# k2-fsa/Flow2GAN

Hardware: AMD Instinct MI355X
Metric: audio-seconds/sec (train step, G+D fwd/bwd) mel_24k_base (higher is better)
Workload: dtype f32 (fp32-class products on the bf16 matrix pipe for the long reductions and the direct MRD convs: every fp32 operand as three bf16 pieces = 24 significand bits, the six v_mfma_f32_32x32x16_bf16 products with i + j <= 2 per fp32 product, fp32 accumulate, error <= 2^-23 per product; short reductions ; 1 GPU; mel_24k_base GAN stage-2 train step: D-step + G-step, each on its own batch (MPD+MRD+FM+multi-scale mel), fwd+bwd+grad all-reduce, no optimizer (metric is fwd/bwd); per_gpu_batch=64, gan=gan_multi_scale_mel_recon, parallelism=dp1, optimizer=none

## Files before the change

### flow2gan_amd/_lib.py

```python
from __future__ import annotations

import ctypes as C
import os

import torch

_HERE = os.path.dirname(os.path.abspath(__file__))
LIB_PATH = os.environ.get("F2G_LIB_PATH") or os.path.join(_HERE, "libflow2gan_hip.so")

c_float_p = C.c_void_p


class Operand(C.Structure):
    _fields_ = [
        ("base", C.c_void_p), ("rows", C.c_int32), ("cols", C.c_int32),
        ("P1", C.c_int32), ("P0", C.c_int32), ("seglen", C.c_int32),
        ("step1", C.c_int32), ("pad1", C.c_int32), ("L1", C.c_int32),
        ("step0", C.c_int32), ("pad0", C.c_int32), ("unit", C.c_int32), ("L0u", C.c_int32),
        ("seq_stride", C.c_int64), ("line_stride", C.c_int64),
        ("reflect", C.c_int32), ("split", C.c_int32),
        ("alpha", C.c_void_p), ("lrelu_src", C.c_void_p),
        ("lrelu_slope", C.c_float), ("unbounded", C.c_int32),
    ]


class Epilogue(C.Structure):
    _fields_ = [
        ("C", C.c_void_p), ("ldc", C.c_int64), ("P0o", C.c_int32), ("c_bf16", C.c_int32),
        ("seq_stride_o", C.c_int64), ("row_stride_o", C.c_int64), ("off_o", C.c_int64),
        ("bias", C.c_void_p), ("res", C.c_void_p), ("ldres", C.c_int64), ("gamma", C.c_void_p),
        ("aux", C.c_void_p), ("ldaux", C.c_int64), ("alpha_n", C.c_void_p),
        ("colsum_alpha", C.c_void_p), ("colsum", C.c_void_p),
        ("lrelu_slope", C.c_float), ("scale", C.c_float),
        ("accumulate", C.c_int32), ("atomic", C.c_int32),
        ("prelu_slope", C.c_void_p), ("prelu_out", C.c_void_p), ("ld_prelu_out", C.c_int64),
        ("mask_src", C.c_void_p), ("fm_ref", C.c_void_p), ("fm_wdev", C.c_void_p),
        ("mask_slope", C.c_float), ("fm_w", C.c_float),
        ("x3_out", C.c_void_p), ("colsum_part_ld", C.c_int64),
    ]


class MultiEntry(C.Structure):
    _fields_ = [("out", C.c_void_p), ("inp", C.c_void_p), ("kind", C.c_int32), ("blocks", C.c_int32),
                ("n", C.c_int32 * 4), ("s", C.c_int64 * 4)]


MULTI_MAX = 48


class MultiDesc(C.Structure):
    _fields_ = [("n", C.c_int32), ("_pad", C.c_int32), ("e", MultiEntry * MULTI_MAX)]


class GemmDesc(C.Structure):
    _fields_ = [("A", Operand), ("B", Operand), ("E", Epilogue), ("form", C.c_int32),
                ("split_k", C.c_int32), ("precision", C.c_int32), ("_pad3", C.c_int32)]


class DwnormFwd(C.Structure):
    _fields_ = [
        ("x", C.c_void_p), ("ldx", C.c_int64), ("z", C.c_void_p), ("ldz", C.c_int64),
        ("B", C.c_int32), ("F", C.c_int32), ("C", C.c_int32), ("K", C.c_int32),
        ("lens", C.c_void_p), ("w_dw", C.c_void_p), ("b_dw", C.c_void_p), ("beta", C.c_void_p),
        ("log_scale", C.c_void_p), ("cproj", C.c_void_p), ("ldcp", C.c_int64),
        ("Fc", C.c_int32), ("up", C.c_int32), ("te", C.c_void_p), ("ldte", C.c_int64),
        ("rstd", C.c_void_p), ("z_format", C.c_int32), ("_pad", C.c_int32),
    ]


class DwnormBwd(C.Structure):
    _fields_ = [
# ... 128 lines not shown
    "f2g_period_fold_bwd": [_P, _P, _I, _I, _I, _I, _I],
    "f2g_fill": [_P, _F, _L],
    "f2g_bucket_arm": [_P, _L, C.c_int32],
    "f2g_scale": [_P, _F, _L],
    "f2g_log_clip": [_P, _L, _F],
    "f2g_conv32_s2_fwd": [C.POINTER(Conv32Desc)],
    "f2g_conv32_s2_dgrad": [C.POINTER(Conv32Desc)],
    "f2g_conv33_fwd": [C.POINTER(Conv32Desc)],
    "f2g_conv33_wgrad": [C.POINTER(Conv32Desc), _P],
    "f2g_conv32_s2_wgrad": [C.POINTER(Conv32Desc), _P],
    "f2g_conv2ch_fwd": [C.POINTER(Conv2chDesc)],
    "f2g_conv2ch_wgrad": [C.POINTER(Conv2chDesc)],
    "f2g_conv2ch_dgrad": [C.POINTER(Conv2chDesc)],
    "f2g_convpost_fwd": [C.POINTER(Conv2chDesc)],
    "f2g_convpost_wgrad": [C.POINTER(Conv2chDesc)],
    "f2g_convpost_dgrad": [C.POINTER(Conv2chDesc)],
    "f2g_wave_stats": [_P, _L, _L, _I, _I, _P, _P],
    "f2g_wave_gain": [_P, _L, _P, _L, _L, _I, _I, _I, _P, _P, _P],
    "f2g_sadam_stats": [_P, _P, _I, _P, _I],
    "f2g_sadam_prepare": [_P, C.POINTER(SadamGroup), _P, _P, _P, _P],
    "f2g_lrelu_bwd_colsum": [_P, _P, _P, _F, _P, _F, _I, _I, _L, _P],
    "f2g_zero_halo": [_P, _I, _I, _I, _I, _I],
    "f2g_sadam_update": [_P, _P, _I, _P],
    "f2g_mlp_pack": [_P, _P, _L, _P, _L, _I, _I],
    "f2g_fused_mlp": [C.POINTER(FusedMlpDesc)],
    "f2g_fused_block": [C.POINTER(DwnormFwd), C.POINTER(FusedMlpDesc)],
    "f2g_fused_block_multi": [C.POINTER(DwnormFwd), C.POINTER(FusedMlpDesc), C.c_int32],
    "f2g_istft_ola_multi": [C.POINTER(OlaMultiDesc), _P, _I, _I, _F, _I],
    "f2g_split_bf16x3": [_P, _P, _L, _I, _I],
    "f2g_multi": [C.POINTER(MultiDesc)],
}
EXPORTS = sorted(list(_SIGS) + ["f2g_version", "f2g_last_error", "f2g_gemm_last_path", "f2g_gemm_last_kernel",
                                 "f2g_fused_last_launch",
                                 "f2g_gemm_lean_ok", "f2g_gemm_wgrad_lean", "f2g_fused_mlp_ok",
                                 "f2g_dwnorm_bwd_workspace", "f2g_split_bf16x3_bytes", "f2g_gemm_x6_ok",
                                 "f2g_gemm_colsum_part_rows", "f2g_set_option", "f2g_get_option",
                                 "f2g_dwconv_bwd_workspace", "f2g_sadam_chunk_elems"])


class F2GError(RuntimeError):
    pass


def _load():
    if not os.path.exists(LIB_PATH):
        raise ImportError(
            f"{LIB_PATH} is missing: build it with `python -c 'import __graft_entry__ as g; "
            "g.build()'` (or `make -C flow2gan_amd/csrc`). There is no CPU fallback.")
    lib = C.CDLL(LIB_PATH)
    for name, args in _SIGS.items():
        fn = getattr(lib, name)
        fn.argtypes = list(args) + [C.c_void_p]
        fn.restype = C.c_int
    for name in ("f2g_dwnorm_bwd_workspace", "f2g_dwconv_bwd_workspace"):
        fn = getattr(lib, name)
        fn.argtypes = [C.c_int32] * 4
        fn.restype = C.c_int64
    lib.f2g_gemm_lean_ok.argtypes = [C.POINTER(GemmDesc)]
    lib.f2g_gemm_lean_ok.restype = C.c_int
    lib.f2g_gemm_wgrad_lean.argtypes = [C.POINTER(GemmDesc)]
    lib.f2g_gemm_wgrad_lean.restype = C.c_int
    lib.f2g_split_bf16x3_bytes.argtypes = [C.c_int32, C.c_int32]
    lib.f2g_split_bf16x3_bytes.restype = C.c_int64
    lib.f2g_gemm_x6_ok.argtypes = [C.POINTER(GemmDesc)]
    lib.f2g_gemm_x6_ok.restype = C.c_int
    lib.f2g_gemm_colsum_part_rows.argtypes = [C.POINTER(GemmDesc)]
    lib.f2g_gemm_colsum_part_rows.restype = C.c_int32
    lib.f2g_fused_mlp_ok.argtypes = [C.c_int32, C.c_int32]
    lib.f2g_fused_mlp_ok.restype = C.c_int
    lib.f2g_sadam_chunk_elems.argtypes = []
    lib.f2g_sadam_chunk_elems.restype = C.c_int32
    lib.f2g_set_option.argtypes = [C.c_char_p, C.c_int32]
    lib.f2g_set_option.restype = C.c_int
    lib.f2g_get_option.argtypes = [C.c_char_p, C.POINTER(C.c_int32)]
    lib.f2g_get_option.restype = C.c_int
    lib.f2g_version.restype = C.c_char_p
    lib.f2g_last_error.restype = C.c_char_p
    lib.f2g_gemm_last_kernel.argtypes = []
    lib.f2g_gemm_last_kernel.restype = C.c_char_p
    lib.f2g_fused_last_launch.argtypes = []
    lib.f2g_fused_last_launch.restype = C.c_char_p
    return lib


lib = _load()


def version() -> str:
    return lib.f2g_version().decode()


def set_option(name: str, value: int) -> int:
    old = C.c_int32()
    if lib.f2g_get_option(name.encode(), C.byref(old)) or lib.f2g_set_option(name.encode(), int(value)):
# ... 45 lines not shown
```

### flow2gan_amd/csrc/capi.hip

```cpp
#include <stdio.h>
#include <stdlib.h>
#include <string.h>
#include <strings.h>

#include <mutex>

#include "common.h"
#include "version_gen.h"

static char g_err[256] = "";

void f2g_set_error(const char* msg) {
  strncpy(g_err, msg ? msg : "", sizeof(g_err) - 1);
  g_err[sizeof(g_err) - 1] = 0;
}

int f2g_check_launch() {
  hipError_t e = hipGetLastError();
  if (e != hipSuccess) {
    f2g_set_error(hipGetErrorString(e));
    return F2G_ELAUNCH;
  }
  return F2G_OK;
}

extern "C" const char* f2g_version(void) { return "flow2gan_hip 0.4.0 src:" F2G_SRC_HASH " gfx950"; }
extern "C" const char* f2g_last_error(void) { return g_err; }

namespace {
struct Opt { const char* name; int value; };
Opt g_opts[F2G_OPT_COUNT] = {
    {"lean_tall", 1}, {"lean_wgrad", 1}, {"x6p", 1}, {"deterministic", 0}, {"streamk", 1}, {"mlp_rt", 0},
    {"mlp_split", 0}, {"multi_rt384", 4}, {"multi_rt512", 3}, {"streamk_min", 4}};
std::once_flag g_opts_once;

int opt_index(const char* name, size_t len) {
  for (int i = 0; i < F2G_OPT_COUNT; ++i)
    if (strlen(g_opts[i].name) == len && strncasecmp(g_opts[i].name, name, len) == 0) return i;
  return -1;
}

void opts_init() {
  const char* e = getenv("F2G_OPTS");
  while (e && *e) {
    const char* end = strchr(e, ',');
    const size_t len = end ? (size_t)(end - e) : strlen(e);
    const char* eq = (const char*)memchr(e, '=', len);
    if (eq) {
      const int i = opt_index(e, (size_t)(eq - e));
      if (i >= 0) g_opts[i].value = atoi(eq + 1);
    }
    e = end ? end + 1 : nullptr;
  }
  const char* det = getenv("F2G_DETERMINISTIC");
  if (det) g_opts[F2G_OPT_DETERMINISTIC].value = atoi(det) != 0;
}
}

int f2g_opt(int id) {
  std::call_once(g_opts_once, opts_init);
  return g_opts[id].value;
}

extern "C" int f2g_set_option(const char* name, int32_t value) {
  std::call_once(g_opts_once, opts_init);
  const int i = name ? opt_index(name, strlen(name)) : -1;
// ... 16 lines not shown
```

### flow2gan_amd/csrc/common.h

```cpp
#pragma once
#include <hip/hip_runtime.h>
#include <stdint.h>

#include <type_traits>

#include "../../include/flow2gan_hip.h"

int f2g_check_launch();
void f2g_note_kernel(const char* name, int split, int path);
enum f2g_opt_id {
  F2G_OPT_LEAN_TALL,
  F2G_OPT_LEAN_WGRAD,
  F2G_OPT_X6P,
  F2G_OPT_DETERMINISTIC,
  F2G_OPT_STREAMK,
  F2G_OPT_MLP_RT,
  F2G_OPT_MLP_SPLIT,
  F2G_OPT_MULTI_RT384,
  F2G_OPT_MULTI_RT512,
  F2G_OPT_STREAMK_MIN,
  F2G_OPT_COUNT
};
int f2g_opt(int id);
int f2g_gemm_narrow(const f2g_gemm_desc& d, hipStream_t st);
void f2g_set_error(const char* msg);
int f2g_x6p_ok(const f2g_gemm_desc& d, int taps);
int f2g_launch_x6p(const f2g_gemm_desc& d, int taps, long long a_extent, hipStream_t st);
int f2g_leanw6t_ok(const f2g_gemm_desc& d, int split);
int f2g_launch_leanw6t(const f2g_gemm_desc& d, int split, hipStream_t st);
struct f2g_colsegs {
  float* out[3];
  int begin[3];
  int count[3];
};
int f2g_colsum_segments(const float* a, long long lda, int rows, int ncols,
                        const f2g_colsegs& segs, hipStream_t st);

#define F2G_WAVE 64

__device__ __forceinline__ float wave_sum(float v) {
#pragma unroll
  for (int o = 32; o > 0; o >>= 1) v += __shfl_xor(v, o);
  return v;
}

__device__ __forceinline__ float wave_max(float v) {
#pragma unroll
  for (int o = 32; o > 0; o >>= 1) v = fmaxf(v, __shfl_xor(v, o));
  return v;
}

typedef float f2g_f32x2 __attribute__((ext_vector_type(2)));
typedef __bf16 f2g_bf16x2 __attribute__((ext_vector_type(2)));
// ... 26 lines not shown
```

### flow2gan_amd/csrc/gemm.hip

```cpp
#include <hip/hip_runtime.h>
#include <stddef.h>
#include <stdint.h>
#include <stdio.h>
#include <string.h>

#include "gemm_common.h"

namespace {

int g_last_path = 0;
const char* g_last_kernel = "";
int g_last_split = 1;

struct RowCtx {
  long long base;
  int l1b, e0;
};

__device__ __forceinline__ RowCtx decode_row(const f2g_operand& S, int r) {
  RowCtx rc;
  int s, p1, p0;
  if (S.P0 == 1 && S.P1 == 1) {
    s = r; p1 = 0; p0 = 0;
  } else {
// ... 720 lines not shown
extern "C" int f2g_to_bf16(void* dst, const float* src, int64_t n, f2g_stream_t stream) {
  if (!dst || !src || (n & 3) || (((uintptr_t)dst) & 7) || !al16(src)) return F2G_EINVAL;
  if (n == 0) return F2G_OK;
  const long long n4 = n / 4;
  long long blocks = (n4 + 255) / 256;
  if (blocks > 256 * 16) blocks = 256 * 16;
  hipLaunchKernelGGL(to_bf16_kernel, dim3((unsigned)blocks), dim3(256), 0, (hipStream_t)stream,
                     reinterpret_cast<uint2*>(dst), reinterpret_cast<const float4*>(src), n4);
  return f2g_check_launch();
}

extern "C" int f2g_split_bf16(float* dst, const float* src, int64_t n, f2g_stream_t stream) {
  if (!dst || !src || (n & 3) || !al16(dst) || !al16(src)) return F2G_EINVAL;
  if (n == 0) return F2G_OK;
  const long long n4 = n / 4;
  long long blocks = (n4 + 255) / 256;
  if (blocks > 256 * 16) blocks = 256 * 16;
  hipLaunchKernelGGL(split_bf16_kernel, dim3((unsigned)blocks), dim3(256), 0, (hipStream_t)stream,
                     reinterpret_cast<uint4*>(dst), reinterpret_cast<const float4*>(src), n4);
  return f2g_check_launch();
}

extern "C" int f2g_gemm(const f2g_gemm_desc* dp, f2g_stream_t stream) {
  if (!dp || !dp->A.base || !dp->B.base || !dp->E.C) return F2G_EINVAL;
  f2g_note_kernel("", 1, g_last_path);
  const f2g_gemm_desc& d = *dp;
  hipStream_t st = (hipStream_t)stream;
  int split = d.split_k > 0 ? d.split_k : 1;
  if (d.E.colsum_part_ld > 0 && f2g_gemm_colsum_part_rows(dp) == 0) {
    f2g_set_error("f2g_gemm: E.colsum_part_ld needs a precision-3 launch with the wide epilogue "
                  "(f2g_gemm_colsum_part_rows(d) == 0 for this descriptor)");
    return F2G_EINVAL;
  }
  if (d.precision == 3 && d.form == 2) {
    if (d.A.split || d.B.split || d.A.rows != d.B.rows || !f2g_leanw_ok(d) || d.E.x3_out ||
        (split > 1 && !d.E.atomic)) {
      f2g_set_error("f2g_gemm precision 3, form 2: fp32 operands the K-major weight-gradient kernel reads");
      return F2G_EINVAL;
    }
    return f2g_launch_leanw(d, 6, split, st);
  }
  if (d.precision == 3) return f2g_gemm_x6(d, st);
  if (d.E.x3_out) {
    f2g_set_error("f2g_gemm: E.x3_out belongs to precision 3");
    return F2G_EINVAL;
  }
  {
    const int nr = f2g_gemm_narrow(d, st);
    if (nr != 0) return nr < 0 ? nr : F2G_OK;
    f2g_note_kernel("", 1, 0);
  }
  if (d.E.prelu_slope && (d.E.atomic || d.E.accumulate || d.E.P0o > 0 || d.form == 2)) return F2G_EINVAL;
  if (d.E.mask_src && (d.E.atomic || d.E.accumulate || d.form == 2)) return F2G_EINVAL;
  if (d.form == 0 || d.form == 1) {
    const bool f1 = d.form == 1;
    if (f1 ? d.A.cols != d.B.rows : d.A.cols != d.B.cols) return F2G_EINVAL;
    if (!host_plain(d.B)) return F2G_EINVAL;
    const int M = d.A.rows, N = f1 ? d.B.cols : d.B.rows, K = d.A.cols;
    const int am = op_mode(d.A, true), bm = op_mode(d.B, !f1);
    const bool linear = d.E.lrelu_slope == 0.f && d.E.res != d.E.C && d.E.aux != d.E.C && !d.E.prelu_slope &&
                        !d.E.mask_src;
    int s = d.split_k;
    const bool no_auto = f2g_opt(F2G_OPT_DETERMINISTIC) != 0;
    const bool presplit = d.A.split != 0 && d.B.split == d.A.split;
    const bool bf16img = d.A.split == 2;
    const bool lean = !f1 && N > 64 && f2g_lean_operands_ok(d) &&
                      (d.precision == 0 || ((d.precision == 1 || d.precision == 2) && presplit)) &&
                      (!bf16img || (d.precision == 2 && f2g_lean_bf16_ok(d)));
    if ((d.A.split || d.B.split) && !(lean && d.precision != 0)) return F2G_EINVAL;
// ... 52 lines not shown
```

### flow2gan_amd/csrc/gemm_common.h

```cpp
#pragma once
#include "common.h"

bool f2g_lean_operands_ok(const f2g_gemm_desc& d);
bool f2g_lean_bf16_ok(const f2g_gemm_desc& d);
int f2g_lean_stream_k(int M, int N, int K, bool all_grids);
int f2g_launch_lean(const f2g_gemm_desc& d, int M, int N, int K, int split, int upb, hipStream_t st);
bool f2g_leanw_ok(const f2g_gemm_desc& d);
bool f2g_leanw_fp32_takes(const f2g_gemm_desc& d, int split);
int f2g_launch_leanw(const f2g_gemm_desc& d, int pieces, int split, hipStream_t st);
int f2g_gemm_x6(const f2g_gemm_desc& d, hipStream_t st);

#ifndef F2G_LABVAR
#define F2G_LABVAR 0
#endif
#ifndef F2G_X6LAB
#define F2G_X6LAB 0
#endif
#if F2G_X6LAB & 1
#define X6LAB_EPI if (acc[0][0][0] == 1.2345e30f)
#else
#define X6LAB_EPI
#endif
#if F2G_X6LAB & 2
#define X6LAB_X3 acc[0][0][1] == 1.2345e30f &&
#else
#define X6LAB_X3
#endif
#if F2G_X6LAB & 256
#define X6PROF_STAMP(t) asm volatile("s_memtime %0" : "=s"(t) : : "memory")
#define X6PROF_ACC(sum, t1, t0)                                                                              \
  {                                                                                                          \
    unsigned dt_;                                                                                            \
    asm volatile("s_sub_u32 %0, %1, %2" : "=s"(dt_) : "s"((unsigned)(t1)), "s"((unsigned)(t0)) : "memory"); \
    sum += dt_;                                                                                              \
  }
#else
#define X6PROF_STAMP(t)
#define X6PROF_ACC(sum, t1, t0)
#endif

namespace {

// ... 140 lines not shown
```

### flow2gan_amd/csrc/gemm_wgrad.hip

```cpp
#include <stddef.h>
#include <stdint.h>

#include "gemm_common.h"

namespace {


template <bool BWIN>
__global__ __launch_bounds__(256, 2)
void gemm_leanw3_kernel(const f2g_gemm_desc d, int M, int N, int K, int kchunk) {
  constexpr int PL = 32 * 256;
  constexpr int BUF = 4 * PL;
  extern __shared__ __attribute__((aligned(16))) float smem[];
  unsigned char* sm = reinterpret_cast<unsigned char*>(smem);
  const int tid = threadIdx.x, lane = tid & 63, wave = tid >> 6;
  const int wm = wave >> 1, wn = wave & 1, li = lane & 31, h = lane >> 5;
  int m0, n0;
  tile_of_block(128, 128, m0, n0);
  const int kbeg = blockIdx.z * kchunk;
  int kend = kbeg + kchunk;
  if (kend > K) kend = K;
  const int nt = (kend - kbeg + BK - 1) / BK;
  if (nt <= 0) return;

// ... 451 lines not shown
  return (long long)(B.rows / B.P0) * B.seq_stride * 4 < 0x7ff00000ll;
}

bool f2g_leanw_fp32_takes(const f2g_gemm_desc& d, int split) {
  const int leanw_mode = f2g_opt(F2G_OPT_LEAN_WGRAD);
  if (d.form != 2 || d.A.split || d.B.split || split < 1) return false;
  return leanw_mode > 0 && d.precision == 0 && d.E.atomic && f2g_leanw_ok(d) &&
         (host_plain(d.B) || d.B.P0 >= 16) && (leanw_mode > 1 || d.A.rows / split >= 4096);
}

template <auto KPLAIN, auto KWIN, int SMEM, int PATH>
static int launch_leanw(const f2g_gemm_desc& d, const char* plain_name, const char* win_name, int split,
                        hipStream_t st) {
  const int M = d.A.cols, N = d.B.cols, K = d.A.rows;
  int kchunk = ((K + split - 1) / split + BK - 1) / BK * BK;
  const int zs = (K + kchunk - 1) / kchunk;
  dim3 grid(M / 128, N / 128, zs);
  dyn_lds_once<KPLAIN, KWIN>(SMEM);
  const bool plain = host_plain(d.B);
  f2g_note_kernel(plain ? plain_name : win_name, split, PATH);
  hipLaunchKernelGGL(plain ? KPLAIN : KWIN, grid, dim3(256), SMEM, st, d, M, N, K, kchunk);
  return f2g_check_launch();
}

int f2g_launch_leanw(const f2g_gemm_desc& d, int pieces, int split, hipStream_t st) {
  if (pieces == 1)
    return launch_leanw<gemm_leanw_kernel<false>, gemm_leanw_kernel<true>, 2 * 2 * 32 * 128 * 4, 1>(
        d, "leanw<bwin=0>", "leanw<bwin=1>", split, st);
  if (pieces == 3)
    return launch_leanw<gemm_leanw3_kernel<false>, gemm_leanw3_kernel<true>, 2 * 4 * 32 * 256, 1>(
        d, "leanw3<bwin=0>", "leanw3<bwin=1>", split, st);
  if (f2g_leanw6t_ok(d, split))
    return f2g_launch_leanw6t(d, split, st);
  return launch_leanw<gemm_leanw6_kernel<false>, gemm_leanw6_kernel<true>, 6 * 32 * 256, 4>(
      d, "leanw6<bwin=0>", "leanw6<bwin=1>", split, st);
}

extern "C" int f2g_gemm_wgrad_lean(const f2g_gemm_desc* dp) {
  if (!dp || !dp->A.base || !dp->B.base) return 0;
  return f2g_leanw_fp32_takes(*dp, dp->split_k < 1 ? 1 : dp->split_k) ? 1 : 0;
}
```

### flow2gan_amd/fused.py

```python
from __future__ import annotations

import os
import random
from typing import List, Optional

import torch

from . import ops
from .models.modules import dft_matrices
from .ops import gemm, mat, win1d

LIMIT_PROB = 0.6


def _limit_draw(training: bool) -> bool:
    return bool(training and random.random() < LIMIT_PROB)


def frames_lens(audio_lens_cpu: Optional[List[int]], hop: int, device):
    if audio_lens_cpu is None:
        return None
    return torch.tensor([1 + int(l) // hop for l in audio_lens_cpu], dtype=torch.int32,
                        device=device)

# ... 93 lines not shown
    zsplit = 1 if fmt == 1 else 0
    z = ops.empty(rows, Cc, device=dev)
    ops.dwnorm_fwd(x, z, B, F, Cc, bp.K, lens, bp.w_dw, bp.b_dw, bp.beta, bp.log_scale.reshape(1),
                   cproj, ldcp, Fc, up, cp_off, te, ldte, te_off, z_format=zsplit)
    a = ops.empty(rows, Hh, device=dev)
    if keep:
        p = ops.empty(rows, Hh, device=dev)
        share = ops.split_sharing(z, p)
        with share:
            gemm(mat(z, rows, Cc, split=zsplit), mat(bp.w1.reshape(Hh, Cc)), a, bias=bp.b1,
                 prelu=bp.alpha, prelu_out=p)
            out = ops.empty(rows, Cc, device=dev)
            gemm(mat(p, rows, Hh), mat(bp.w2.reshape(Cc, Hh)), out, bias=bp.b2, res=x,
                 gamma=bp.gamma.reshape(Cc))
        return out, z, (a, p, share, zsplit)
    p = a
    gemm(mat(z, rows, Cc, split=zsplit), mat(bp.w1.reshape(Hh, Cc)), a, bias=bp.b1, prelu=bp.alpha)
    out = ops.empty(rows, Cc, device=dev)
    gemm(mat(p, rows, Hh), mat(bp.w2.reshape(Cc, Hh)), out, bias=bp.b2, res=x,
         gamma=bp.gamma.reshape(Cc))
    return out, z, (a, p, None, zsplit)


def block_bwd(bp: _Blk, x, z, a, gout, B, F, lens, limit_norm: bool, limit_scale: bool,
              cproj=None, ldcp=0, Fc=0, up=1, cp_off=0, te=None, ldte=0, te_off=0, g_cproj=None,
              g_te=None, g_cproj_store=False):
    a, p_act, share, zsplit = a
    if share is None:
        share = ops.split_sharing()
    dev = x.device
    rows, Cc, Hh = B * F, bp.C, bp.H
    (g_w2, g_b2, g_alpha, g_b1, g_w1, g_beta, g_ls, g_wdw, g_bdw, g_gamma) = ops.zeros_many(
        [(Cc, Hh), (Cc,), (Hh,), (Hh,), (Hh, Cc), (Cc,), (1,), (Cc, 1, bp.K), (Cc,), (Cc, 1)], dev)
    ops.colsum(g_b2, gout, rows, Cc)
    with share, ops.split_sharing(gout):
        ops.wgrad(gout, Cc, gout.stride(0), mat(p_act, rows, Hh), g_w2)
        gemm(mat(gout, rows, Cc), mat(bp.w2.reshape(Cc, Hh)), a, form=1, aux=a, alpha_n=bp.alpha,
             colsum_alpha=g_alpha, colsum=g_b1)
    with share, ops.split_sharing(a):
        ops.wgrad(a, Hh, a.stride(0), mat(z, rows, Cc, split=zsplit), g_w1)
        gemm(mat(a, rows, Hh), mat(bp.w1.reshape(Hh, Cc)), z, form=1)
    share.drop()
    du = ops.empty(rows, Cc, device=dev)
    ops.dwnorm_bwd(x, z, du, B, F, Cc, bp.K, lens, bp.w_dw, bp.b_dw, bp.beta,
                   bp.log_scale.reshape(1), cproj, ldcp, Fc, up, cp_off, te, ldte, te_off,
                   g_cproj=g_cproj, g_te=g_te, g_beta=g_beta, g_log_scale=g_ls,
                   g_cproj_store=g_cproj_store)
    gx = ops.empty(rows, Cc, device=dev)
    ops.dwconv_bwd(du, x, gx, B, F, Cc, bp.K, lens, bp.w_dw, gres=gout, gamma=bp.gamma.reshape(Cc),
                   g_w=g_wdw, g_b=g_bdw, g_gamma=g_gamma)
    if limit_norm:
        ops.limit_grad(g_ls, bp.log_scale.reshape(1), -1.5, 1.5)
    if limit_scale:
        ops.limit_grad(g_gamma, bp.gamma, 0.5, 1.0)
    grads = [g_wdw, g_bdw, g_ls.reshape(()), g_beta, g_w1.reshape(Hh, Cc, 1), g_b1, g_alpha,
             g_w2.reshape(Cc, Hh, 1), g_b2, g_gamma]
    return gx, grads


def cond_encoder_params(enc) -> list:
    p = [enc.in_proj.weight, enc.in_proj.bias, enc.in_norm.log_scale, enc.in_norm.bias]
    for blk in enc.blocks:
        p += block_params(blk)
    return p


class CondEncoderFn(GradAwareFunction):

    @staticmethod
# ... 758 lines not shown
```

### flow2gan_amd/ops.py

```python
from __future__ import annotations

import ctypes as C
from typing import Optional

import torch

from . import _lib as L
from ._opts import opt
from ._lib import DwconvBwd, DwnormBwd, DwnormFwd, Epilogue, GemmDesc, Operand, call, ptr


def empty(*shape, device, dtype=torch.float32):
    return torch.empty(*shape, device=device, dtype=dtype)


def zeros(*shape, device):
    t = torch.empty(*shape, device=device, dtype=torch.float32)
    fill_(t, 0.0)
    return t


def fill_(t, v: float):
    if BATCH is not None and t.numel() > 0:
        import struct
# ... 325 lines not shown
    o.lrelu_slope = slope
    o.unbounded = 1 if (unbounded and offset == 0 and t.is_contiguous()
                        and t.numel() == nseq * o.seq_stride) else 0
    o._keep = (t, lrelu_src)
    return o


def win2d(t, nseq: int, H: int, W: int, Cin: int, W_out: int, kh: int, kw: int, stride_w: int,
          pad_h: int, pad_w: int, line_stride: Optional[int] = None,
          seq_stride: Optional[int] = None, offset: int = 0, lrelu_src=None,
          slope: float = 0.0) -> Operand:
    o = Operand()
    o.base = ptr(t) + 4 * offset
    o.rows, o.cols = nseq * H * W_out, kh * kw * Cin
    o.P1, o.P0 = H, W_out
    o.seglen = kw * Cin
    o.step1, o.pad1, o.L1 = 1, pad_h, H
    o.step0, o.pad0, o.unit, o.L0u = stride_w, pad_w, Cin, W * Cin
    o.line_stride = line_stride if line_stride is not None else W * Cin
    o.seq_stride = seq_stride if seq_stride is not None else H * o.line_stride
    o.reflect = 0
    o.alpha = None
    o.lrelu_src = None if lrelu_src is None else ptr(lrelu_src) + 4 * offset
    o.lrelu_slope = slope
    o._keep = (t, lrelu_src)
    return o


def gemm(A: Operand, Bm: Operand, out, form: int = 0, ldc: Optional[int] = None, *, bias=None,
         res=None, ldres: Optional[int] = None, gamma=None, aux=None, ldaux: Optional[int] = None,
         alpha_n=None, colsum_alpha=None, colsum=None, lrelu: float = 0.0, scale: float = 0.0,
         accumulate: bool = False, atomic: bool = False, split_k: int = 0, out_offset: int = 0,
         rowmap=None, prelu=None, prelu_out=None, mask=None, fm=None, x3_out: bool = False,
         true_k: Optional[int] = None, true_n: Optional[int] = None):
    if form == 1:
        src = getattr(Bm, "_src", None)
        if src is not None and src.shape[0] % 32 == 0 and src.shape[1] > 64:
            Bm, form = mat(transposed(src)), 0
    d = GemmDesc()
    d.A, d.B = A, Bm
    e = Epilogue()
    e.C = ptr(out) + 4 * out_offset
    e.ldc = ldc if ldc is not None else out.stride(0)
    e.c_bf16 = 1 if out.dtype == torch.bfloat16 else 0
    if rowmap is not None:
        e.P0o, e.seq_stride_o, e.row_stride_o, e.off_o = rowmap
    else:
        e.P0o = 0
    e.bias = ptr(bias)
    e.res = ptr(res)
    e.ldres = ldres if ldres is not None else (res.stride(0) if res is not None else 0)
    e.gamma = ptr(gamma)
    e.aux = ptr(aux)
    e.ldaux = ldaux if ldaux is not None else (aux.stride(0) if aux is not None else 0)
    e.alpha_n = ptr(alpha_n)
    e.colsum_alpha = ptr(colsum_alpha)
    e.colsum = ptr(colsum)
    e.lrelu_slope = lrelu
    e.scale = scale
    e.accumulate = 1 if accumulate else 0
    e.atomic = 1 if atomic else 0
    e.prelu_slope = ptr(prelu)
    e.prelu_out = ptr(prelu_out)
    e.ld_prelu_out = prelu_out.stride(0) if prelu_out is not None else 0
    if mask is not None:
        e.mask_src = ptr(mask[0]) + 4 * mask[1]
        e.mask_slope = float(mask[2])
        if fm is not None:
            e.fm_ref = ptr(fm[0]) + 4 * fm[1]
            e.fm_w = float(fm[2])
            e.fm_wdev = ptr(fm[3])
    d.E = e
    d.form = form
    if split_k == -1:
        tiles = ((A.cols + 127) // 128) * ((Bm.cols + 127) // 128)
        split_k = split_for(A.rows, tiles)
        if form == 2 and GEMM_PRECISION == 0 and atomic:
            d.split_k, d.precision = split_k, 0
            if L.lib.f2g_gemm_wgrad_lean(C.byref(d)):
                split_k = split_for(A.rows, tiles, True)
    d.split_k = split_k
    d.precision = GEMM_PRECISION
    if GEMM_PRECISION == 3:
        d.precision = 0
        in_kernel = X6F == 1
        if X6F == 2 and X6F_MIN_K <= A.cols < X6_MIN_K and (
                (Bm.rows >= X6F_MIN_N and ((A.rows + 127) // 128) * ((Bm.rows + 127) // 128) >= X6F_MIN_TILES)
                or (A.rows >= X6F_TALL_ROWS and Bm.rows >= 128)):
            in_kernel = True
        if X6F == 2 and 128 <= A.cols < X6_MIN_K and A.rows >= X6F_TALL_ROWS and Bm.rows == 32:
            in_kernel = True
        if X6F == 2 and X6_MIN_K <= A.cols < X6_NOPASS_K and A.P0 == 1 and A.P1 == 1 and not _is_const(A._keep[0]):
            in_kernel = True
        if form == 0 and A.split == 0 and Bm.split == 0 and A.rows >= X6_MIN_ROWS \
                and (A.cols >= X6_MIN_K or in_kernel) and not atomic \
                and split_k <= 1 and out.dtype == torch.float32 and _x3_window_ok(A):
            buf = getattr(out, "_f2g_x3_buf", None) if x3_out else None
            if buf is not None and X6F != 1 and not getattr(out, "_f2g_x3_bad", False) \
                    and out_offset % 32 == 0 and prelu_out is None:
                d.E.x3_out = ptr(buf) + (out_offset // 32) * 192
            how = L.lib.f2g_gemm_x6_ok(C.byref(d))
            if not how and d.E.x3_out:
                d.E.x3_out = None
                how = L.lib.f2g_gemm_x6_ok(C.byref(d))
            if how:
                if in_kernel and not (how & 4):
                    in_kernel = False
                    how = how if A.cols >= X6_MIN_K else 0
                if how:
                    if not in_kernel:
                        d.A, d.B = _x3_operand(A), _x3_operand(Bm)
                    elif Bm.P0 == 1 and Bm.P1 == 1 and _is_const(Bm._keep[0]):
                        d.B = _x3_operand(Bm, frag_major=X6G and Bm.rows % 32 == 0 and Bm.rows > 32)
                    d.precision = 3
            if d.precision != 3:
                d.E.x3_out = None
        if form == 2 and atomic and A.split == 0 and Bm.split == 0 and A.lrelu_src is None \
                and A.rows >= X6_MIN_K and L.lib.f2g_gemm_lean_ok(C.byref(d)):
            d.precision = 3
        if x3_out:
            if d.E.x3_out:
                out._f2g_x3 = out._f2g_x3_buf
            else:
                out._f2g_x3_bad = True
    if (GEMM_PRECISION == 1 and form in (0, 2)) or (GEMM_PRECISION == 2 and form == 0):
        ok = L.lib.f2g_gemm_lean_ok(C.byref(d))
        if GEMM_PRECISION == 2 and (ok & 2):
            d.A, d.B = _bf16_operand(A), _bf16_operand(Bm)
        elif ok:
            d.A, d.B = _split_operand(A), _split_operand(Bm)
    parts = None
    if COLSUM_PARTS and d.precision == 3 and form == 0 and (colsum is not None or colsum_alpha is not None) \
            and A.rows >= COLSUM_PARTS_MIN_ROWS:
        nrows = L.lib.f2g_gemm_colsum_part_rows(C.byref(d))
        if nrows > 0:
            ncol = Bm.rows
            both = colsum is not None and colsum_alpha is not None
            parts = torch.empty(nrows, (2 if both else 1) * ncol, device=out.device, dtype=torch.float32)
            d.E.colsum_part_ld = parts.stride(0)
            if colsum_alpha is not None:
                d.E.colsum_alpha = ptr(parts)
            if colsum is not None:
                d.E.colsum = ptr(parts) + (4 * ncol if both else 0)
    if GEMM_TIMER is not None:
        GEMM_TIMER.launch(d, A, Bm, form, true_k, true_n)
    else:
        call("f2g_gemm", C.byref(d))
    if parts is not None:
        nrows, ncol = parts.shape[0], Bm.rows
        if colsum is not None and colsum_alpha is not None and ptr(colsum) == ptr(colsum_alpha) + 4 * ncol:
            call("f2g_colsum", ptr(colsum_alpha), ptr(parts), parts.stride(0), None, 0, nrows, 2 * ncol)
            return out
# ... 594 lines not shown
    def join(self):
        if not self.on:
            return
        for s in self.streams:
            ev = torch.cuda.Event()
            ev.record(s)
            self.main.wait_event(ev)


def split_for(reduction_rows: int, out_tiles: int, two_per_cu: bool = False) -> int:
    slabs = max(1, reduction_rows // 32)
    smax = max(1, min(512, slabs // 16))
    R = 256
    if two_per_cu:
        R = 512
        smax = max(1, min(smax, reduction_rows // 4096))
    cands = set(range(1, min(smax, 64) + 1))
    for m in range(1, 9):
        s = (R * m) // out_tiles
        if 1 <= s <= smax:
            cands.add(s)

    def fill(s):
        b = out_tiles * s
        return b / (((b + R - 1) // R) * R)

    best = max(fill(s) for s in cands)
    pair = [s for s in cands if out_tiles * s <= 512 and fill(s) >= best - 0.05]
    if pair:
        return max(pair)
    return min(s for s in cands if fill(s) >= best - 0.02)


def wgrad(dY, M: int, ldy: int, X: Operand, g_out, ldg: Optional[int] = None, out_offset: int = 0,
          dy_lrelu_src=None, slope: float = 0.0):
    rows = X.rows
    A = mat(dY, rows, M, ldy, lrelu_src=dy_lrelu_src, slope=slope)
    gemm(A, X, g_out, form=2, ldc=ldg, atomic=True, split_k=-1, out_offset=out_offset)


def fused_mlp_applies(Cc: int, Hh: int) -> bool:
    return GEMM_PRECISION == 2 and bool(L.lib.f2g_fused_mlp_ok(Cc, Hh))


def mlp_pack(w1, w2):
    def build(ts):
        a, b = ts
        Hh, Cc = a.shape[0], a.shape[1]
        out = torch.empty(2 * Cc * Hh, device=a.device, dtype=torch.bfloat16)
        call("f2g_mlp_pack", ptr(out), ptr(a), Cc, ptr(b), Hh, Cc, Hh)
        return out
    return derived_multi([w1, w2], "mlp_pack", build)


def fused_mlp(z, wp, b1, alpha, b2, res, gamma, out, rows: int, Cc: int, Hh: int, parts: int = 0):
    d = L.FusedMlpDesc()
    d.parts = parts
    d.z, d.ldz, d.wp = ptr(z), z.stride(0), ptr(wp)
    d.b1, d.alpha, d.b2 = ptr(b1), ptr(alpha), ptr(b2)
    d.res, d.ldres, d.gamma = ptr(res), (res.stride(0) if res is not None else 0), ptr(gamma)
    d.out, d.ldo = ptr(out), out.stride(0)
    d.rows, d.C, d.H = rows, Cc, Hh
    if GEMM_TIMER is not None:
        GEMM_TIMER.time(lambda: call("f2g_fused_mlp", C.byref(d)), 4.0 * rows * Cc * Hh,
                        (0, rows, Cc, 2 * Hh), path="fused-mlp")
    else:
        call("f2g_fused_mlp", C.byref(d))
    return out


def fused_block(x, B, F, Cc, K, lens, w_dw, b_dw, beta, log_scale, wp, b1, alpha, b2, gamma, out,
# ... 495 lines not shown
```

### include/flow2gan_hip.h

```cpp
#ifndef FLOW2GAN_HIP_H
#define FLOW2GAN_HIP_H

#include <stdint.h>

#ifdef __cplusplus
extern "C" {
#endif

typedef void* f2g_stream_t;

enum {
  F2G_OK = 0,
  F2G_EINVAL = -1,
  F2G_ELAUNCH = -2,
};

const char* f2g_version(void);
const char* f2g_last_error(void);

int f2g_set_option(const char* name, int32_t value);
int f2g_get_option(const char* name, int32_t* value);

typedef struct {
  const float* base;
// ... 10 lines not shown
  float lrelu_slope;
  int32_t unbounded;
} f2g_operand;

typedef struct {
  float* C;
  int64_t ldc;
  int32_t P0o;
  int32_t c_bf16;
  int64_t seq_stride_o, row_stride_o, off_o;
  const float* bias;
  const float* res;
  int64_t ldres;
  const float* gamma;
  const float* aux;
  int64_t ldaux;
  const float* alpha_n;
  float* colsum_alpha;
  float* colsum;
  float lrelu_slope;
  float scale;
  int32_t accumulate;
  int32_t atomic;
  const float* prelu_slope;
  float* prelu_out;
  int64_t ld_prelu_out;
  const float* mask_src;
  const float* fm_ref;
  const float* fm_wdev;
  float mask_slope;
  float fm_w;
  void* x3_out;
  int64_t colsum_part_ld;
} f2g_epilogue;

typedef struct {
  f2g_operand A, B;
  f2g_epilogue E;
  int32_t form;
  int32_t split_k;
  int32_t precision;
  int32_t _pad3;
} f2g_gemm_desc;

int f2g_gemm(const f2g_gemm_desc* d, f2g_stream_t stream);
int f2g_gemm_wgrad_lean(const f2g_gemm_desc* d);
int f2g_gemm_lean_ok(const f2g_gemm_desc* d);
int f2g_split_bf16(float* dst, const float* src, int64_t n, f2g_stream_t stream);
int f2g_to_bf16(void* dst, const float* src, int64_t n, f2g_stream_t stream);
int64_t f2g_split_bf16x3_bytes(int32_t rows, int32_t K);
int f2g_split_bf16x3(void* dst, const float* src, int64_t ld, int32_t rows, int32_t K, f2g_stream_t stream);
int f2g_gemm_x6_ok(const f2g_gemm_desc* d);
int32_t f2g_gemm_colsum_part_rows(const f2g_gemm_desc* d);

int f2g_gemm_last_path(void);
const char* f2g_gemm_last_kernel(void);

typedef struct {
  const float* x;
  int64_t ldx;
  float* z;
  int64_t ldz;
  int32_t B, F, C, K;
  const int32_t* lens;
  const float* w_dw;
  const float* b_dw;
  const float* beta;
  const float* log_scale;
  const float* cproj;
  int64_t ldcp;
  int32_t Fc, up;
  const float* te;
  int64_t ldte;
  float* rstd;
  int32_t z_format;
  int32_t _pad;
} f2g_dwnorm_fwd_desc;
int f2g_dwnorm_fwd(const f2g_dwnorm_fwd_desc* d, f2g_stream_t stream);

// ... 303 lines not shown
```

Measured before the change: 786.5 audio-s/s.

## Add wide-tile bf16x3 weight-gradient kernel with fused A column-sum

Adds a new weight-gradient GEMM kernel that uses larger output tiles (256x256 or 192x384 per 512-thread block) with in-kernel three-way bf16 splitting, LDS double buffering and six MFMA products per fp32 product. It also folds the bias-gradient column sum of dY into the kernel, so the MLP backward no longer runs a separate colsum pass over gout. Split-K is re-chosen from the wide tile count. The aim is more operand reuse per load and one fewer read of dY, at the cost of higher register and LDS use per block (launch bounds of one block) and atomic adds on the outputs.

Result: no change. 791.1 audio-s/s (median of 6 runs) (+0.6%).

```diff
diff --git a/flow2gan_amd/_lib.py b/flow2gan_amd/_lib.py
--- a/flow2gan_amd/_lib.py
+++ b/flow2gan_amd/_lib.py
@@ -36,7 +36,7 @@
         ("prelu_slope", C.c_void_p), ("prelu_out", C.c_void_p), ("ld_prelu_out", C.c_int64),
         ("mask_src", C.c_void_p), ("fm_ref", C.c_void_p), ("fm_wdev", C.c_void_p),
         ("mask_slope", C.c_float), ("fm_w", C.c_float),
-        ("x3_out", C.c_void_p), ("colsum_part_ld", C.c_int64),
+        ("x3_out", C.c_void_p), ("colsum_part_ld", C.c_int64), ("colsum_a", C.c_void_p),
     ]
 
 
@@ -231,7 +231,7 @@
 }
 EXPORTS = sorted(list(_SIGS) + ["f2g_version", "f2g_last_error", "f2g_gemm_last_path", "f2g_gemm_last_kernel",
                                  "f2g_fused_last_launch",
-                                 "f2g_gemm_lean_ok", "f2g_gemm_wgrad_lean", "f2g_fused_mlp_ok",
+                                 "f2g_gemm_lean_ok", "f2g_gemm_wgrad_lean", "f2g_gemm_wgrad_wide", "f2g_fused_mlp_ok",
                                  "f2g_dwnorm_bwd_workspace", "f2g_split_bf16x3_bytes", "f2g_gemm_x6_ok",
                                  "f2g_gemm_colsum_part_rows", "f2g_set_option", "f2g_get_option",
                                  "f2g_dwconv_bwd_workspace", "f2g_sadam_chunk_elems"])
@@ -259,6 +259,8 @@
     lib.f2g_gemm_lean_ok.restype = C.c_int
     lib.f2g_gemm_wgrad_lean.argtypes = [C.POINTER(GemmDesc)]
     lib.f2g_gemm_wgrad_lean.restype = C.c_int
+    lib.f2g_gemm_wgrad_wide.argtypes = [C.POINTER(GemmDesc)]
+    lib.f2g_gemm_wgrad_wide.restype = C.c_int32
     lib.f2g_split_bf16x3_bytes.argtypes = [C.c_int32, C.c_int32]
     lib.f2g_split_bf16x3_bytes.restype = C.c_int64
     lib.f2g_gemm_x6_ok.argtypes = [C.POINTER(GemmDesc)]
diff --git a/flow2gan_amd/csrc/capi.hip b/flow2gan_amd/csrc/capi.hip
--- a/flow2gan_amd/csrc/capi.hip
+++ b/flow2gan_amd/csrc/capi.hip
@@ -31,7 +31,8 @@
 struct Opt { const char* name; int value; };
 Opt g_opts[F2G_OPT_COUNT] = {
     {"lean_tall", 1}, {"lean_wgrad", 1}, {"x6p", 1}, {"deterministic", 0}, {"streamk", 1}, {"mlp_rt", 0},
-    {"mlp_split", 0}, {"multi_rt384", 4}, {"multi_rt512", 3}, {"streamk_min", 4}};
+    {"mlp_split", 0}, {"multi_rt384", 4}, {"multi_rt512", 3}, {"streamk_min", 4},
+    {"wgrad_wide", 1}};
 std::once_flag g_opts_once;
 
 int opt_index(const char* name, size_t len) {
diff --git a/flow2gan_amd/csrc/common.h b/flow2gan_amd/csrc/common.h
--- a/flow2gan_amd/csrc/common.h
+++ b/flow2gan_amd/csrc/common.h
@@ -19,6 +19,7 @@
   F2G_OPT_MULTI_RT384,
   F2G_OPT_MULTI_RT512,
   F2G_OPT_STREAMK_MIN,
+  F2G_OPT_WGRAD_WIDE,
   F2G_OPT_COUNT
 };
 int f2g_opt(int id);
diff --git a/flow2gan_amd/csrc/gemm.hip b/flow2gan_amd/csrc/gemm.hip
--- a/flow2gan_amd/csrc/gemm.hip
+++ b/flow2gan_amd/csrc/gemm.hip
@@ -776,9 +776,14 @@
                   "(f2g_gemm_colsum_part_rows(d) == 0 for this descriptor)");
     return F2G_EINVAL;
   }
+  if (d.E.colsum_a && !(d.precision == 3 && d.form == 2 && f2g_leanw6w_tiles(d, split) > 0)) {
+    f2g_set_error("f2g_gemm: E.colsum_a needs a launch the wide weight-gradient kernel takes "
+                  "(f2g_gemm_wgrad_wide(d) > 0 for this descriptor)");
+    return F2G_EINVAL;
+  }
   if (d.precision == 3 && d.form == 2) {
-    if (d.A.split || d.B.split || d.A.rows != d.B.rows || !f2g_leanw_ok(d) || d.E.x3_out ||
-        (split > 1 && !d.E.atomic)) {
+    if (d.A.split || d.B.split || d.A.rows != d.B.rows || d.E.x3_out || (split > 1 && !d.E.atomic) ||
+        (!f2g_leanw_ok(d) && f2g_leanw6w_tiles(d, split) == 0)) {
       f2g_set_error("f2g_gemm precision 3, form 2: fp32 operands the K-major weight-gradient kernel reads");
       return F2G_EINVAL;
     }
diff --git a/flow2gan_amd/csrc/gemm_common.h b/flow2gan_amd/csrc/gemm_common.h
--- a/flow2gan_amd/csrc/gemm_common.h
+++ b/flow2gan_amd/csrc/gemm_common.h
@@ -8,6 +8,8 @@
 bool f2g_leanw_ok(const f2g_gemm_desc& d);
 bool f2g_leanw_fp32_takes(const f2g_gemm_desc& d, int split);
 int f2g_launch_leanw(const f2g_gemm_desc& d, int pieces, int split, hipStream_t st);
+int f2g_leanw6w_tiles(const f2g_gemm_desc& d, int split);
+int f2g_launch_leanw6w(const f2g_gemm_desc& d, int split, hipStream_t st);
 int f2g_gemm_x6(const f2g_gemm_desc& d, hipStream_t st);
 
 #ifndef F2G_LABVAR
diff --git a/flow2gan_amd/csrc/gemm_wgrad.hip b/flow2gan_amd/csrc/gemm_wgrad.hip
--- a/flow2gan_amd/csrc/gemm_wgrad.hip
+++ b/flow2gan_amd/csrc/gemm_wgrad.hip
@@ -507,6 +507,8 @@
         d, "leanw3<bwin=0>", "leanw3<bwin=1>", split, st);
   if (f2g_leanw6t_ok(d, split))
     return f2g_launch_leanw6t(d, split, st);
+  if (f2g_leanw6w_tiles(d, split) > 0)
+    return f2g_launch_leanw6w(d, split, st);
   return launch_leanw<gemm_leanw6_kernel<false>, gemm_leanw6_kernel<true>, 6 * 32 * 256, 4>(
       d, "leanw6<bwin=0>", "leanw6<bwin=1>", split, st);
 }
diff --git a/flow2gan_amd/csrc/gemm_wgrad_wide.hip b/flow2gan_amd/csrc/gemm_wgrad_wide.hip
--- /dev/null
+++ b/flow2gan_amd/csrc/gemm_wgrad_wide.hip
@@ -0,0 +1,204 @@
+#include <stddef.h>
+#include <stdint.h>
+
+#include "gemm_common.h"
+
+namespace {
+
+template <int TM, int TN>
+__global__ __launch_bounds__(512, 1) void gemm_leanw6w_kernel(const f2g_gemm_desc d, int K, int kchunk) {
+  constexpr int BMT = 64 * TM, BNT = 128 * TN;
+  constexpr int PA = (BMT + 127) / 128, PB = BNT / 128;
+  constexpr int PLB = 16 * 256;
+  constexpr int OFFB = PA * 3 * PLB;
+  constexpr int BUFB = (PA + PB) * 3 * PLB;
+  extern __shared__ __attribute__((aligned(16))) unsigned char smw[];
+  const int tid = threadIdx.x, lane = tid & 63, wave = tid >> 6;
+  const int wm = wave >> 2, wn = wave & 3, li = lane & 31, h = lane >> 5;
+  int m0, n0;
+  tile_of_block(BMT, BNT, m0, n0);
+  const int kbeg = blockIdx.z * kchunk;
+  int kend = kbeg + kchunk;
+  if (kend > K) kend = K;
+  const int nt = (kend - kbeg + 15) / 16;
+  if (nt <= 0) return;
+  __amdgpu_buffer_rsrc_t ra = __builtin_amdgcn_make_buffer_rsrc(
+      (void*)d.A.base, 0, (unsigned)((long long)K * d.A.seq_stride * 4), 0x00020000);
+  __amdgpu_buffer_rsrc_t rb = __builtin_amdgcn_make_buffer_rsrc(
+      (void*)d.B.base, 0, (unsigned)((long long)K * d.B.seq_stride * 4), 0x00020000);
+  const int cc = tid & 31, r0 = tid >> 5;
+  const unsigned offA = (unsigned)(((long long)r0 * d.A.seq_stride + m0 + 4 * cc) * 4);
+  const unsigned offB = (unsigned)(((long long)r0 * d.B.seq_stride + n0 + 4 * cc) * 4);
+  const int rowA = (int)(d.A.seq_stride * 4), rowB = (int)(d.B.seq_stride * 4);
+  const int wof = r0 * 256 + ((((cc >> 3) ^ (r0 & 3))) << 6) + (cc & 7) * 8;
+  const int g4 = lane >> 4, i16 = lane & 15;
+  const int rrow = (g4 >> 1) * 8 + (i16 >> 2), within = (g4 & 1) * 32 + (i16 & 3) * 8;
+  int rofA[TM], rofB[TN];
+#pragma unroll
+  for (int mi = 0; mi < TM; ++mi) {
+    const int cb = wm * TM + mi;
+    rofA[mi] = (cb >> 2) * 3 * PLB + rrow * 256 + ((((cb & 3) ^ (rrow & 3))) << 6) + within;
+  }
+#pragma unroll
+  for (int ni = 0; ni < TN; ++ni) {
+    const int cb = wn * TN + ni;
+    rofB[ni] = OFFB + (cb >> 2) * 3 * PLB + rrow * 256 + ((((cb & 3) ^ (rrow & 3))) << 6) + within;
+  }
+  f32x16 acc[TM][TN];
+#pragma unroll
+  for (int mi = 0; mi < TM; ++mi)
+#pragma unroll
+    for (int ni = 0; ni < TN; ++ni)
+#pragma unroll
+      for (int e = 0; e < 16; ++e) acc[mi][ni][e] = 0.f;
+  float cs[PA][4];
+#pragma unroll
+  for (int p = 0; p < PA; ++p)
+#pragma unroll
+    for (int j = 0; j < 4; ++j) cs[p][j] = 0.f;
+
+  u32x4 xa[PA], xb[PB];
+  auto gload = [&](int s) {
+    const int s_ = s < nt ? s : 0;
+    const unsigned past = (unsigned)(kbeg + s * 16 + r0 >= kend) << 31;
+    const int soA = (kbeg + s_ * 16) * rowA, soB = (kbeg + s_ * 16) * rowB;
+#pragma unroll
+    for (int p = 0; p < PA; ++p) xa[p] = __builtin_amdgcn_raw_buffer_load_b128(ra, (offA + p * 512) | past, soA, 0);
+#pragma unroll
+    for (int p = 0; p < PB; ++p) xb[p] = __builtin_amdgcn_raw_buffer_load_b128(rb, (offB + p * 512) | past, soB, 0);
+  };
+  auto stageA = [&](unsigned char* buf, int p) {
+    u32x2 p0, p1, p2;
+    const u32x4 v = xa[p];
+    cs[p][0] += __uint_as_float(v.x);
+    cs[p][1] += __uint_as_float(v.y);
+    cs[p][2] += __uint_as_float(v.z);
+    cs[p][3] += __uint_as_float(v.w);
+    split3x4(v, p0, p1, p2);
+    unsigned char* q = buf + p * 3 * PLB + wof;
+    *reinterpret_cast<u32x2*>(q) = p0;
+    *reinterpret_cast<u32x2*>(q + PLB) = p1;
+    *reinterpret_cast<u32x2*>(q + 2 * PLB) = p2;
+  };
+  auto stageB = [&](unsigned char* buf, int p) {
+    u32x2 p0, p1, p2;
+    split3x4(xb[p], p0, p1, p2);
+    unsigned char* q = buf + OFFB + p * 3 * PLB + wof;
+    *reinterpret_cast<u32x2*>(q) = p0;
+    *reinterpret_cast<u32x2*>(q + PLB) = p1;
+    *reinterpret_cast<u32x2*>(q + 2 * PLB) = p2;
+  };
+  auto stage = [&](unsigned char* buf, int c) {
+    if (c < PA) stageA(buf, c);
+    else stageB(buf, c - PA);
+  };
+  constexpr int NCH = PA + PB;
+  gload(0);
+#pragma unroll
+  for (int c = 0; c < NCH; ++c) stage(smw, c);
+  gload(1);
+  lds_barrier();
+  for (int s = 0; s < nt; ++s) {
+    const unsigned char* cur = smw + (s & 1) * BUFB;
+    unsigned char* nxt = smw + ((s + 1) & 1) * BUFB;
+    bf16x8 fa[3][TM];
+#pragma unroll
+    for (int pc = 0; pc < 3; ++pc)
+#pragma unroll
+      for (int mi = 0; mi < TM; ++mi) fa[pc][mi] = tr_frag(cur + pc * PLB + rofA[mi]);
+#pragma unroll
+    for (int ni = 0; ni < TN; ++ni) {
+      bf16x8 fb[3];
+#pragma unroll
+      for (int pc = 0; pc < 3; ++pc) fb[pc] = tr_frag(cur + pc * PLB + rofB[ni]);
+#pragma unroll
+      for (int c = ni * NCH / TN; c < (ni + 1) * NCH / TN; ++c) stage(nxt, c);
+#pragma unroll
+      for (int sdeg = 2; sdeg >= 0; --sdeg)
+#pragma unroll
+        for (int i = 0; i < 3; ++i) {
+          const int j = sdeg - i;
+          if (j < 0 || j > 2) continue;
+#pragma unroll
+          for (int mi = 0; mi < TM; ++mi)
+            acc[mi][ni] = __builtin_amdgcn_mfma_f32_32x32x16_bf16(fa[i][mi], fb[j], acc[mi][ni], 0, 0, 0);
+        }
+    }
+    gload(s + 2);
+    lds_barrier();
+  }
+  if (d.E.colsum_a && n0 == 0) {
+    float* red = reinterpret_cast<float*>(smw);
+#pragma unroll
+    for (int p = 0; p < PA; ++p)
+      *reinterpret_cast<float4*>(red + r0 * (PA * 128) + p * 128 + 4 * cc) =
+          make_float4(cs[p][0], cs[p][1], cs[p][2], cs[p][3]);
+    __syncthreads();
+    if (tid < BMT) {
+      float v = 0.f;
+#pragma unroll
+      for (int r = 0; r < 16; ++r) v += red[r * (PA * 128) + tid];
+      atomicAdd(d.E.colsum_a + m0 + tid, v);
+    }
+  }
+  float* C0 = d.E.C;
+#pragma unroll
+  for (int mi = 0; mi < TM; ++mi)
+#pragma unroll
+    for (int ni = 0; ni < TN; ++ni)
+#pragma unroll
+      for (int e = 0; e < 16; ++e) {
+        const int row = m0 + (wm * TM + mi) * 32 + (e & 3) + 8 * (e >> 2) + 4 * h;
+        atomicAdd(C0 + (long long)row * d.E.ldc + n0 + (wn * TN + ni) * 32 + li, acc[mi][ni][e]);
+      }
+}
+
+template <int TM, int TN>
+int launch_wide(const f2g_gemm_desc& d, const char* name, int split, hipStream_t st) {
+  constexpr int BMT = 64 * TM, BNT = 128 * TN;
+  constexpr size_t smem = (size_t)2 * ((BMT + 127) / 128 + BNT / 128) * 3 * 16 * 256;
+  const int M = d.A.cols, N = d.B.cols, K = d.A.rows;
+  dyn_lds_once<gemm_leanw6w_kernel<TM, TN>>((int)smem);
+  const int kchunk = ((K + split - 1) / split + 15) / 16 * 16;
+  const int zs = (K + kchunk - 1) / kchunk;
+  dim3 grid(M / BMT, N / BNT, zs);
+  f2g_note_kernel(name, split, 4);
+  hipLaunchKernelGGL((gemm_leanw6w_kernel<TM, TN>), grid, dim3(512), smem, st, d, K, kchunk);
+  return f2g_check_launch();
+}
+
+int wide_instance(const f2g_gemm_desc& d, int split) {
+  const int mode = f2g_opt(F2G_OPT_WGRAD_WIDE);
+  const f2g_epilogue& E = d.E;
+  if (mode == 0 || d.form != 2 || d.precision != 3 || split < 1 || d.A.split || d.B.split) return 0;
+  const f2g_operand& A = d.A;
+  const f2g_operand& B = d.B;
+  if (A.rows != B.rows || A.rows <= 0 || !host_plain(A) || !host_plain(B) || A.alpha || B.alpha) return 0;
+  if (!al16(A.base) || !al16(B.base) || (A.seq_stride & 3) || (B.seq_stride & 3)) return 0;
+  if ((long long)A.rows * A.seq_stride * 4 >= 0x7ff00000ll || (long long)B.rows * B.seq_stride * 4 >= 0x7ff00000ll) return 0;
+  if (!E.atomic || E.P0o > 0 || E.bias || E.res || (E.scale != 0.f && E.scale != 1.f) || E.colsum || E.colsum_alpha ||
+      E.lrelu_slope != 0.f || E.mask_src || E.aux || E.prelu_slope || E.c_bf16 || E.x3_out || E.accumulate)
+    return 0;
+  const int M = d.A.cols, N = d.B.cols;
+  const int inst = (M % 256 == 0 && N % 256 == 0) ? 1 : (M % 192 == 0 && N % 384 == 0) ? 2 : 0;
+  if (inst == 0 || mode > 1) return inst;
+  return (d.A.rows >= 4096 && d.A.rows / split >= 256) ? inst : 0;
+}
+
+}
+
+int f2g_leanw6w_tiles(const f2g_gemm_desc& d, int split) {
+  const int inst = wide_instance(d, split);
+  if (inst == 0) return 0;
+  return inst == 1 ? (d.A.cols / 256) * (d.B.cols / 256) : (d.A.cols / 192) * (d.B.cols / 384);
+}
+
+int f2g_launch_leanw6w(const f2g_gemm_desc& d, int split, hipStream_t st) {
+  if (wide_instance(d, split) == 1) return launch_wide<4, 2>(d, "leanw6w<tm=4,tn=2>", split, st);
+  return launch_wide<3, 3>(d, "leanw6w<tm=3,tn=3>", split, st);
+}
+
+extern "C" int32_t f2g_gemm_wgrad_wide(const f2g_gemm_desc* dp) {
+  if (!dp || !dp->A.base || !dp->B.base) return 0;
+  return f2g_leanw6w_tiles(*dp, dp->split_k < 1 ? 1 : dp->split_k);
+}
diff --git a/flow2gan_amd/fused.py b/flow2gan_amd/fused.py
--- a/flow2gan_amd/fused.py
+++ b/flow2gan_amd/fused.py
@@ -149,9 +149,8 @@
     rows, Cc, Hh = B * F, bp.C, bp.H
     (g_w2, g_b2, g_alpha, g_b1, g_w1, g_beta, g_ls, g_wdw, g_bdw, g_gamma) = ops.zeros_many(
         [(Cc, Hh), (Cc,), (Hh,), (Hh,), (Hh, Cc), (Cc,), (1,), (Cc, 1, bp.K), (Cc,), (Cc, 1)], dev)
-    ops.colsum(g_b2, gout, rows, Cc)
     with share, ops.split_sharing(gout):
-        ops.wgrad(gout, Cc, gout.stride(0), mat(p_act, rows, Hh), g_w2)
+        ops.wgrad(gout, Cc, gout.stride(0), mat(p_act, rows, Hh), g_w2, a_colsum=g_b2)
         gemm(mat(gout, rows, Cc), mat(bp.w2.reshape(Cc, Hh)), a, form=1, aux=a, alpha_n=bp.alpha,
              colsum_alpha=g_alpha, colsum=g_b1)
     with share, ops.split_sharing(a):
diff --git a/flow2gan_amd/ops.py b/flow2gan_amd/ops.py
--- a/flow2gan_amd/ops.py
+++ b/flow2gan_amd/ops.py
@@ -381,7 +381,7 @@
          alpha_n=None, colsum_alpha=None, colsum=None, lrelu: float = 0.0, scale: float = 0.0,
          accumulate: bool = False, atomic: bool = False, split_k: int = 0, out_offset: int = 0,
          rowmap=None, prelu=None, prelu_out=None, mask=None, fm=None, x3_out: bool = False,
-         true_k: Optional[int] = None, true_n: Optional[int] = None):
+         true_k: Optional[int] = None, true_n: Optional[int] = None, colsum_a=None):
     if form == 1:
         src = getattr(Bm, "_src", None)
         if src is not None and src.shape[0] % 32 == 0 and src.shape[1] > 64:
@@ -419,8 +419,11 @@
             e.fm_ref = ptr(fm[0]) + 4 * fm[1]
             e.fm_w = float(fm[2])
             e.fm_wdev = ptr(fm[3])
+    e.colsum_a = ptr(colsum_a)
     d.E = e
     d.form = form
+    w6 = GEMM_PRECISION == 3 and form == 2 and atomic and A.split == 0 and Bm.split == 0 and A.lrelu_src is None \
+        and A.rows >= X6_MIN_K
     if split_k == -1:
         tiles = ((A.cols + 127) // 128) * ((Bm.cols + 127) // 128)
         split_k = split_for(A.rows, tiles)
@@ -428,6 +431,11 @@
             d.split_k, d.precision = split_k, 0
             if L.lib.f2g_gemm_wgrad_lean(C.byref(d)):
                 split_k = split_for(A.rows, tiles, True)
+        if w6:
+            d.split_k, d.precision = split_k, 3
+            wide = L.lib.f2g_gemm_wgrad_wide(C.byref(d))
+            if wide:
+                split_k = split_for(A.rows, wide)
     d.split_k = split_k
     d.precision = GEMM_PRECISION
     if GEMM_PRECISION == 3:
@@ -464,9 +472,10 @@
                     d.precision = 3
             if d.precision != 3:
                 d.E.x3_out = None
-        if form == 2 and atomic and A.split == 0 and Bm.split == 0 and A.lrelu_src is None \
-                and A.rows >= X6_MIN_K and L.lib.f2g_gemm_lean_ok(C.byref(d)):
+        if w6:
             d.precision = 3
+            if not (L.lib.f2g_gemm_wgrad_wide(C.byref(d)) or L.lib.f2g_gemm_lean_ok(C.byref(d))):
+                d.precision = 0
         if x3_out:
             if d.E.x3_out:
                 out._f2g_x3 = out._f2g_x3_buf
@@ -1127,11 +1136,25 @@
     return min(s for s in cands if fill(s) >= best - 0.02)
 
 
+def wgrad_wide_tiles(A: Operand, X: Operand, g_out, ldg: Optional[int] = None, split_k: int = 1) -> int:
+    if not (GEMM_PRECISION == 3 and A.split == 0 and X.split == 0 and A.lrelu_src is None and A.rows >= X6_MIN_K):
+        return 0
+    d = GemmDesc()
+    d.A, d.B = A, X
+    d.E.C, d.E.ldc, d.E.atomic = ptr(g_out), ldg if ldg is not None else g_out.stride(0), 1
+    d.form, d.split_k, d.precision = 2, max(1, split_k), 3
+    return int(L.lib.f2g_gemm_wgrad_wide(C.byref(d)))
+
+
 def wgrad(dY, M: int, ldy: int, X: Operand, g_out, ldg: Optional[int] = None, out_offset: int = 0,
-          dy_lrelu_src=None, slope: float = 0.0):
+          dy_lrelu_src=None, slope: float = 0.0, a_colsum=None):
     rows = X.rows
     A = mat(dY, rows, M, ldy, lrelu_src=dy_lrelu_src, slope=slope)
-    gemm(A, X, g_out, form=2, ldc=ldg, atomic=True, split_k=-1, out_offset=out_offset)
+    if a_colsum is not None and not (dy_lrelu_src is None and wgrad_wide_tiles(A, X, g_out, ldg)):
+        colsum(a_colsum, dY, rows, M)
+        a_colsum = None
+    gemm(A, X, g_out, form=2, ldc=ldg, atomic=True, split_k=-1, out_offset=out_offset,
+         colsum_a=a_colsum)
 
 
 def fused_mlp_applies(Cc: int, Hh: int) -> bool:
diff --git a/include/flow2gan_hip.h b/include/flow2gan_hip.h
--- a/include/flow2gan_hip.h
+++ b/include/flow2gan_hip.h
@@ -66,6 +66,7 @@
   float fm_w;
   void* x3_out;
   int64_t colsum_part_ld;
+  float* colsum_a;
 } f2g_epilogue;
 
 typedef struct {
@@ -79,6 +80,7 @@
 
 int f2g_gemm(const f2g_gemm_desc* d, f2g_stream_t stream);
 int f2g_gemm_wgrad_lean(const f2g_gemm_desc* d);
+int32_t f2g_gemm_wgrad_wide(const f2g_gemm_desc* d);
 int f2g_gemm_lean_ok(const f2g_gemm_desc* d);
 int f2g_split_bf16(float* dst, const float* src, int64_t n, f2g_stream_t stream);
 int f2g_to_bf16(void* dst, const float* src, int64_t n, f2g_stream_t stream);
```
